# Hanbo-Cheng/DAWN-pytorch

Measured on AMD Instinct MI355X. Metric: generated frames/sec at 256x256, 50 DDIM steps, higher is better.
Workload: dtype f32

## Files before the change

dawn-pytorch_amd/csrc/misc.hip:

```cpp
#include "dawn_common.h"
#include "../../include/dawn_hip.h"

namespace {

__global__ __launch_bounds__(256) void init_conv_x_kernel(const float* __restrict__ x, const float* __restrict__ w3,
                                                          const float* __restrict__ fea_pre, int F, int h, int w,
                                                          int Co, float* __restrict__ out, const long plane) {
    extern __shared__ __attribute__((aligned(16))) float ws[];
    for (int i = threadIdx.x; i < 147 * Co; i += 256) ws[i] = w3[i];
    __syncthreads();
    const int tpp = Co >> 2;
    const long npix = (long)F * h * w;
    const long total = npix * tpp;
    for (long t = (long)blockIdx.x * 256 + threadIdx.x; t < total; t += (long)gridDim.x * 256) {
        const long pix = t / tpp;
        const int cq = (int)(t - pix * tpp);
        const int f = (int)(pix / (h * w));
        const int rem = (int)(pix - (long)f * h * w);
        const int y = rem / w, xx = rem - y * w;
        f32x4 acc = *reinterpret_cast<const f32x4*>(fea_pre + (long)rem * Co + cq * 4);
        for (int ky = 0; ky < 7; ++ky) {
            const int yi = y + ky - 3;
            if (yi < 0 || yi >= h) continue;
            for (int kx = 0; kx < 7; ++kx) {
                const int xi = xx + kx - 3;
                if (xi < 0 || xi >= w) continue;
                const long off = ((long)f * h + yi) * w + xi;
#pragma unroll
                for (int c = 0; c < 3; ++c) {
                    const float xv = x[c * plane + off];
                    const f32x4 wv = *reinterpret_cast<const f32x4*>(ws + ((ky * 7 + kx) * 3 + c) * Co + cq * 4);
                    acc += xv * wv;
                }
            }
        }
        *reinterpret_cast<f32x4*>(out + pix * Co + cq * 4) = acc;
    }
}

__global__ __launch_bounds__(256) void init_conv_x_mfma_kernel(const float* __restrict__ x, const float* __restrict__ w3,
                                                               const float* __restrict__ fea_pre, int F, int h, int w,
                                                               float* __restrict__ out, const long plane) {
    extern __shared__ __attribute__((aligned(16))) float sm[];
    constexpr int Co = 64, KP = 148;
    const int TR = 256 / w, PW = w + 6, PS = (TR + 6) * PW;
    float* Ws = sm;
    float* Ps = sm + KP * Co;
    const int tid = threadIdx.x;
    const int tiles_per_frame = h / TR;
    for (int i = tid; i < KP * Co; i += 256) Ws[i] = i < 147 * Co ? w3[i] : 0.f;
    for (int tile = blockIdx.x; tile < F * tiles_per_frame; tile += gridDim.x) {
    const int f = tile / tiles_per_frame;
    const int y0 = (tile - f * tiles_per_frame) * TR;
    __syncthreads();
    for (int i = tid; i < 3 * PS; i += 256) {
        const int c = i / PS, rem = i - c * PS;
        const int py = rem / PW, px = rem - py * PW;
        const int y = y0 + py - 3, xx = px - 3;
        Ps[i] = (y >= 0 && y < h && xx >= 0 && xx < w) ? x[c * plane + ((long)f * h + y) * w + xx] : 0.f;
    }
    __syncthreads();
    const int wave = tid >> 6, lane = tid & 63, l31 = lane & 31, half = lane >> 5;
    f32x16 acc[2][2];
#pragma unroll
    for (int i = 0; i < 2; ++i)
#pragma unroll
        for (int j = 0; j < 2; ++j)
#pragma unroll
            for (int r = 0; r < 16; ++r) acc[i][j][r] = 0.f;
    int pbase[2];
#pragma unroll
    for (int i = 0; i < 2; ++i) {
        const int p = wave * 64 + i * 32 + l31;
        const int ty = p / w, tx = p - ty * w;
        pbase[i] = ty * PW + tx;
    }
#pragma unroll 2
    for (int s = 0; s < KP / 2; ++s) {
        const int k = 2 * s + half;
        const int kk = k < 147 ? k : 0;
        const int tap = kk / 3, c = kk - tap * 3;
        const int ky = tap / 7, kx = tap - ky * 7;
        const int koff = c * PS + ky * PW + kx;
        const float a0 = Ws[k * Co + l31], a1 = Ws[k * Co + 32 + l31];
        const float b0 = Ps[pbase[0] + koff], b1 = Ps[pbase[1] + koff];
        acc[0][0] = __builtin_amdgcn_mfma_f32_32x32x2f32(a0, b0, acc[0][0], 0, 0, 0);
        acc[0][1] = __builtin_amdgcn_mfma_f32_32x32x2f32(a1, b0, acc[0][1], 0, 0, 0);
        acc[1][0] = __builtin_amdgcn_mfma_f32_32x32x2f32(a0, b1, acc[1][0], 0, 0, 0);
        acc[1][1] = __builtin_amdgcn_mfma_f32_32x32x2f32(a1, b1, acc[1][1], 0, 0, 0);
    }
#pragma unroll
    for (int i = 0; i < 2; ++i) {
        const int p = wave * 64 + i * 32 + l31;
        const long rem = (long)y0 * w + p;
        const float* fp = fea_pre + rem * Co;
        float* op = out + ((long)f * h * w + rem) * Co;
#pragma unroll
        for (int j = 0; j < 2; ++j)
#pragma unroll
            for (int g = 0; g < 4; ++g) {
                const int n = 32 * j + 8 * g + 4 * half;
                const f32x4 v = {acc[i][j][4 * g], acc[i][j][4 * g + 1], acc[i][j][4 * g + 2], acc[i][j][4 * g + 3]};
                *reinterpret_cast<f32x4*>(op + n) = v + *reinterpret_cast<const f32x4*>(fp + n);
            }
    }
    }
}

__global__ __launch_bounds__(256) void head_out_kernel(const float* __restrict__ hg, const float* __restrict__ ho,
                                                       const float* __restrict__ wg, const float* __restrict__ bg,
                                                       const float* __restrict__ wo, const float* __restrict__ bo,
                                                       long rows, int Co, float* __restrict__ eps_out) {
    const int sub = threadIdx.x & 15;
    const long row = (long)blockIdx.x * 16 + (threadIdx.x >> 4);
    float a0 = 0.f, a1 = 0.f, a2 = 0.f;
    if (row < rows) {
        for (int c = sub * 4; c < Co; c += 64) {
            if (hg) {
                const f32x4 g = *reinterpret_cast<const f32x4*>(hg + row * Co + c);
                const f32x4 w0 = *reinterpret_cast<const f32x4*>(wg + c);
                const f32x4 w1 = *reinterpret_cast<const f32x4*>(wg + Co + c);
                a0 += g.x * w0.x + g.y * w0.y + g.z * w0.z + g.w * w0.w;
                a1 += g.x * w1.x + g.y * w1.y + g.z * w1.z + g.w * w1.w;
            }
            if (ho) {
                const f32x4 o = *reinterpret_cast<const f32x4*>(ho + row * Co + c);
                const f32x4 w2 = *reinterpret_cast<const f32x4*>(wo + c);
                a2 += o.x * w2.x + o.y * w2.y + o.z * w2.z + o.w * w2.w;
            }
        }
    }
    a0 = wave_sum(a0, 16); a1 = wave_sum(a1, 16); a2 = wave_sum(a2, 16);
    if (row < rows && sub == 0) {
        if (hg) {
            eps_out[row] = a0 + bg[0];
            eps_out[rows + row] = a1 + bg[1];
        }
        if (ho) eps_out[2 * rows + row] = a2 + bo[0];
    }
}

constexpr int HEADS_RPT = 4;
template <int NQ>
__global__ __launch_bounds__(256) void heads_eps_kernel(const float* __restrict__ c2g, const float* __restrict__ a2g, const float* __restrict__ b2g,
                                                        const float* __restrict__ c2o, const float* __restrict__ a2o, const float* __restrict__ b2o,
                                                        const float* __restrict__ in0, int ld0, int C0, const float* __restrict__ in1, int ld1, int C1,
                                                        const float* __restrict__ wg, const float* __restrict__ wo, const float* __restrict__ Wf,
                                                        const float* __restrict__ bf, long rows, int Co, float* __restrict__ eps_out) {
    const int sub = threadIdx.x & 15;
    const long row0 = (long)blockIdx.x * (16 * HEADS_RPT) + (threadIdx.x >> 4);
    const int Cin = C0 + C1;
    const f32x4 z4 = {0.f, 0.f, 0.f, 0.f};
    f32x4 wg0[NQ], wg1[NQ], wo2[NQ], ag[NQ], bgn[NQ], ao[NQ], bon[NQ], f0[NQ][3], f1[NQ][3];
#pragma unroll
    for (int q = 0; q < NQ; ++q) {
        const int c = sub * 4 + 64 * q;
        wg0[q] = wg1[q] = wo2[q] = ag[q] = bgn[q] = ao[q] = bon[q] = z4;
#pragma unroll
        for (int j = 0; j < 3; ++j) f0[q][j] = f1[q][j] = z4;
// ... 41 lines not shown
                const float sg = dawn_silu(vg[i][q][e] * ag[q][e] + bgn[q][e]);
                const float so = dawn_silu(vo[i][q][e] * ao[q][e] + bon[q][e]);
                const float x0 = v0[i][q][e], x1 = v1[i][q][e];
                e0 += sg * wg0[q][e] + x0 * f0[q][0][e] + x1 * f1[q][0][e];
                e1 += sg * wg1[q][e] + x0 * f0[q][1][e] + x1 * f1[q][1][e];
                e2 += so * wo2[q][e] + x0 * f0[q][2][e] + x1 * f1[q][2][e];
            }
        }
        e0 = wave_sum(e0, 16); e1 = wave_sum(e1, 16); e2 = wave_sum(e2, 16);
        if (row < rows && sub == 0) {
            if (c2g) {
                eps_out[row] = e0 + bf[0];
                eps_out[rows + row] = e1 + bf[1];
            }
            if (c2o) eps_out[2 * rows + row] = e2 + bf[2];
        }
    }
}

__global__ __launch_bounds__(256) void linear_kernel(const float* __restrict__ in, int M, int K, int ld_in,
                                                     const float* __restrict__ W, const float* __restrict__ bias, int N,
                                                     int act_in, float* __restrict__ out, int ld_out) {
    const long o = (long)blockIdx.x * 4 + (threadIdx.x >> 6);
    if (o >= (long)M * N) return;
    const int lane = threadIdx.x & 63;
    const int m = (int)(o / N), n = (int)(o - (long)m * N);
    float acc = 0.f;
    for (int k = lane; k < K; k += 64) {
        float v = in[(long)m * ld_in + k];
        if (act_in == 1) v = dawn_silu(v);
        else if (act_in == 2) v = 0.5f * v * (1.0f + erff(v * 0.70710678118654752f));
        acc += v * W[(long)n * K + k];
    }
    acc = wave_sum(acc);
    if (lane == 0) out[(long)m * ld_out + n] = acc + (bias ? bias[n] : 0.f);
}

__global__ void sinusoidal_kernel(float t, int dim, const float* __restrict__ freqs, float* __restrict__ out) {
    const int i = threadIdx.x;
    const int half = dim / 2;
    if (i < half) {
        const float a = __fmul_rn(t, freqs[i]);
        out[i] = sinf(a);
        out[half + i] = cosf(a);
    }
}

}

extern "C" int dawn_init_conv_x_ex(const float* x, long plane_stride, const float* w3, const float* fea_pre, int F, int h, int w, int Co,
                                   float* out, void* stream) {
    if (plane_stride < (long)F * h * w) return dawn_set_error_msg(-61, "dawn_init_conv_x: plane stride smaller than a plane");
    if (Co % 4 != 0 || 147 * Co * 4 > 60000) return dawn_set_error_msg(-60, "dawn_init_conv_x: bad Co");
    if (Co == 64 && w <= 256 && 256 % w == 0 && h % (256 / w) == 0 && (256 / w) <= h) {
        const int TR = 256 / w;
        const int lds = (148 * 64 + 3 * (TR + 6) * (w + 6)) * (int)sizeof(float);
        const int ntiles = F * (h / TR);
        const int slots = 3 * 256;
        hipLaunchKernelGGL(init_conv_x_mfma_kernel, dim3(ntiles < slots ? ntiles : slots), dim3(256), lds, (hipStream_t)stream, x, w3, fea_pre,
                           F, h, w, out, plane_stride);
        DAWN_LAUNCH_CHECK();
        return 0;
    }
    const long total = (long)F * h * w * (Co / 4);
    int grid = (int)((total + 255) / 256);
    if (grid > 4096) grid = 4096;
    hipLaunchKernelGGL(init_conv_x_kernel, dim3(grid), dim3(256), 147 * Co * sizeof(float), (hipStream_t)stream, x, w3,
                       fea_pre, F, h, w, Co, out, plane_stride);
    DAWN_LAUNCH_CHECK();
    return 0;
}
extern "C" int dawn_init_conv_x(const float* x, const float* w3, const float* fea_pre, int F, int h, int w, int Co,
                                float* out, void* stream) {
    return dawn_init_conv_x_ex(x, (long)F * h * w, w3, fea_pre, F, h, w, Co, out, stream);
}
extern "C" int dawn_head_out(const float* hg, const float* ho, const float* wg, const float* bg, const float* wo,
                             const float* bo, long rows, int Co, float* eps_out, void* stream) {
    hipLaunchKernelGGL(head_out_kernel, dim3(dawn_cdiv(rows, 16)), dim3(256), 0, (hipStream_t)stream, hg, ho, wg, bg,
                       wo, bo, rows, Co, eps_out);
    DAWN_LAUNCH_CHECK();
    return 0;
}
extern "C" int dawn_heads_eps(const float* c2g, const float* a2g, const float* b2g, const float* c2o, const float* a2o, const float* b2o,
                              const float* in0, int ld0, int C0, const float* in1, int ld1, int C1, const float* wg, const float* wo,
                              const float* Wf, const float* bf, long rows, int Co, float* eps_out, void* stream) {
    if (Co <= 0 || Co % 4 != 0 || C0 <= 0 || C0 % 4 != 0 || C1 < 0 || C1 % 4 != 0 || ld0 % 4 != 0 || ld1 % 4 != 0 || ld0 < C0 || ld1 < C1)
        return dawn_set_error_msg(-62, "dawn_heads_eps: Co, C0, C1, ld0 and ld1 must be multiples of 4 (ld >= C)");
    if (Co > 256 || C0 > 256 || C1 > 256) return dawn_set_error_msg(-62, "dawn_heads_eps: more than 256 channels in one source");
    if ((!c2g && !c2o) || !in0 || (C1 > 0 && !in1) || !Wf || !bf || !eps_out || (c2g && (!a2g || !b2g || !wg)) || (c2o && (!a2o || !b2o || !wo)))
        return dawn_set_error_msg(-62, "dawn_heads_eps: null argument");
    const uintptr_t al = (uintptr_t)c2g | (uintptr_t)a2g | (uintptr_t)b2g | (uintptr_t)c2o | (uintptr_t)a2o | (uintptr_t)b2o | (uintptr_t)in0 |
                         (uintptr_t)in1 | (uintptr_t)wg | (uintptr_t)wo | (uintptr_t)Wf;
    if (al & 15) return dawn_set_error_msg(-62, "dawn_heads_eps: pointers must be 16-byte aligned");
    if (rows <= 0) return 0;
    const int mc = Co > C0 ? (Co > C1 ? Co : C1) : (C0 > C1 ? C0 : C1);
    const dim3 grid(dawn_cdiv(rows, 16 * HEADS_RPT)), block(256);
#define HEADS_LAUNCH(NQ)                                                                                                              \
    hipLaunchKernelGGL(heads_eps_kernel<NQ>, grid, block, 0, (hipStream_t)stream, c2g, a2g, b2g, c2o, a2o, b2o, in0, ld0, C0, in1, ld1, C1, \
                       wg, wo, Wf, bf, rows, Co, eps_out)
    if (mc <= 64) HEADS_LAUNCH(1);
    else if (mc <= 128) HEADS_LAUNCH(2);
    else HEADS_LAUNCH(4);
#undef HEADS_LAUNCH
    DAWN_LAUNCH_CHECK();
    return 0;
}
extern "C" int dawn_fold_heads(const float* wg, const float* bg, const float* wo, const float* bo, const float* wr_g, const float* br_g,
                               const float* wr_o, const float* br_o, int Co, int Cin, float* Wf, float* bf) {
    if (!wg || !bg || !wo || !bo || !wr_g || !br_g || !wr_o || !br_o || !Wf || !bf || Co <= 0 || Cin <= 0)
        return dawn_set_error_msg(-63, "dawn_fold_heads: null argument or empty shape");
    for (int j = 0; j < 3; ++j) {
        const float* w = j < 2 ? wg + (long)j * Co : wo;
        const float* wr = j < 2 ? wr_g : wr_o;
// ... 59 lines not shown
```

dawn-pytorch_amd/csrc/sampler.hip:

```cpp
#include "dawn_common.h"
#include "../../include/dawn_hip.h"
#include <stdio.h>

namespace {

__global__ __launch_bounds__(256) void ddim_x0_kernel(const float* __restrict__ x, const float* __restrict__ eps,
                                                      float recip, float recipm1, long n, float* __restrict__ x0,
                                                      unsigned* __restrict__ hist) {
    __shared__ unsigned hs[2048];
    for (int i = threadIdx.x; i < 2048; i += 256) hs[i] = 0;
    __syncthreads();
    for (long i = (long)blockIdx.x * 256 + threadIdx.x; i < n; i += (long)gridDim.x * 256) {
        const float v = __fsub_rn(__fmul_rn(recip, x[i]), __fmul_rn(recipm1, eps[i]));
        x0[i] = v;
        const unsigned u = __float_as_uint(v) & 0x7fffffffu;
        atomicAdd(&hs[u >> 20], 1u);
    }
    __syncthreads();
    for (int i = threadIdx.x; i < 2048; i += 256)
        if (hs[i]) atomicAdd(&hist[i], hs[i]);
}

__global__ __launch_bounds__(256) void select_hist_kernel(const float* __restrict__ x0, long n,
                                                          const unsigned* __restrict__ state, int pass,
                                                          unsigned* __restrict__ hist) {
    __shared__ unsigned hs[1024];
    const unsigned prefix = state[0];
    if (pass < 4) {
        for (int i = threadIdx.x; i < 1024; i += 256) hs[i] = 0;
    } else if (threadIdx.x == 0) {
        hs[0] = 0x7fffffffu;
    }
    __syncthreads();
    const int sh = pass == 2 ? 20 : 10;
    for (long i = (long)blockIdx.x * 256 + threadIdx.x; i < n; i += (long)gridDim.x * 256) {
        const unsigned u = __float_as_uint(x0[i]) & 0x7fffffffu;
        if (pass == 4) {
            if (u > prefix) atomicMin(&hs[0], u);
        } else if ((u >> sh) == prefix) {
            atomicAdd(&hs[(pass == 2 ? (u >> 10) : u) & 1023u], 1u);
        }
    }
    __syncthreads();
    if (pass == 4) {
        if (threadIdx.x == 0) atomicMin(&hist[0], hs[0]);
    } else {
        for (int i = threadIdx.x; i < 1024; i += 256)
            if (hs[i]) atomicAdd(&hist[i], hs[i]);
    }
}

__global__ __launch_bounds__(256) void select_scan_kernel(const unsigned* __restrict__ hist, int nbins,
                                                          unsigned long long rank0, unsigned* __restrict__ state,
                                                          int pass) {
    __shared__ unsigned long long part[256];
    const int per = nbins / 256;
    const int t = threadIdx.x;
    unsigned long long s = 0;
    for (int i = 0; i < per; ++i) s += hist[t * per + i];
    part[t] = s;
    __syncthreads();
    if (t == 0) {
        const unsigned long long r = pass == 1 ? rank0 : (unsigned long long)state[1];
        unsigned long long cum = 0;
        int ch = -1;
        for (int i = 0; i < 256; ++i) {
            if (r < cum + part[i]) { ch = i; break; }
            cum += part[i];
        }
        if (ch < 0) { ch = 255; cum -= part[255]; }
        int b = ch * per + per - 1;
        unsigned long long before = cum;
        for (int i = 0; i < per; ++i) {
            const unsigned long long c = hist[ch * per + i];
            if (r < before + c) { b = ch * per + i; break; }
            if (i < per - 1) before += c;
        }
        const unsigned long long rin = r >= before ? r - before : 0;
        const unsigned prefix = pass == 1 ? 0u : state[0];
        state[0] = pass == 1 ? (unsigned)b : ((prefix << 10) | (unsigned)b);
        state[1] = (unsigned)rin;
        state[2] = hist[b];
        state[3] = (rin + 1 < (unsigned long long)hist[b]) ? 1u : 0u;
    }
}

__global__ void select_finalize_kernel(const unsigned* __restrict__ state, const unsigned* __restrict__ hmin,
                                       float weight, float* __restrict__ s_out) {
    if (threadIdx.x == 0 && blockIdx.x == 0) {
        const float lo = __uint_as_float(state[0]);
        float hi = lo;
        if (!state[3] && hmin[0] != 0x7fffffffu) hi = __uint_as_float(hmin[0]);
        const float df = __fsub_rn(hi, lo);
        float q = weight < 0.5f ? __fadd_rn(lo, __fmul_rn(weight, df)) : __fsub_rn(hi, __fmul_rn(df, __fsub_rn(1.0f, weight)));
        s_out[0] = fmaxf(q, 1.0f);
        s_out[1] = q;
    }
}

__global__ __launch_bounds__(256) void ddim_update_kernel(const float* __restrict__ x0, const float* __restrict__ eps,
                                                          const float* __restrict__ sp, const float* __restrict__ noise,
                                                          float san, float c, float sigma, long n,
                                                          float* __restrict__ x) {
    const float s = sp[0];
    for (long i = (long)blockIdx.x * 256 + threadIdx.x; i < n; i += (long)gridDim.x * 256) {
        float v = fminf(fmaxf(x0[i], -s), s) / s;
        float r = __fadd_rn(__fmul_rn(v, san), __fmul_rn(c, eps[i]));
        if (noise) r = __fadd_rn(r, __fmul_rn(sigma, noise[i]));
        x[i] = r;
    }
}

__global__ __launch_bounds__(256) void ancestral_update_kernel(const float* __restrict__ x0, const float* x_t,
                                                               const float* __restrict__ sp, const float* __restrict__ noise,
                                                               float c1, float c2, float std, long n, float* out) {
    const float s = sp[0];
    for (long i = (long)blockIdx.x * 256 + threadIdx.x; i < n; i += (long)gridDim.x * 256) {
        float v = fminf(fmaxf(x0[i], -s), s) / s;
        float r = __fadd_rn(__fmul_rn(v, c1), __fmul_rn(c2, x_t[i]));
        if (noise) r = __fadd_rn(r, __fmul_rn(std, noise[i]));
        out[i] = r;
    }
}

__device__ __forceinline__ void philox_round(unsigned& c0, unsigned& c1, unsigned& c2, unsigned& c3, unsigned k0,
                                             unsigned k1) {
    const unsigned long long p0 = (unsigned long long)0xD2511F53u * c0;
    const unsigned long long p1 = (unsigned long long)0xCD9E8D57u * c2;
    const unsigned n0 = (unsigned)(p1 >> 32) ^ c1 ^ k0;
    const unsigned n1 = (unsigned)p1;
    const unsigned n2 = (unsigned)(p0 >> 32) ^ c3 ^ k1;
    const unsigned n3 = (unsigned)p0;
    c0 = n0; c1 = n1; c2 = n2; c3 = n3;
}

__global__ __launch_bounds__(256) void philox_normal_kernel(float* __restrict__ out, int C, int F, int f0, int Ftotal,
                                                            int hw, unsigned long long seed, unsigned stream_id) {
    const int qpf = hw >> 2;
    const long total = (long)C * F * qpf;
    for (long t = (long)blockIdx.x * 256 + threadIdx.x; t < total; t += (long)gridDim.x * 256) {
        const int qd = (int)(t % qpf);
        const long cf = t / qpf;
        const int f = (int)(cf % F), c = (int)(cf / F);
        const unsigned long long gq = ((unsigned long long)c * Ftotal + (f0 + f)) * qpf + qd;
        unsigned c0 = (unsigned)gq, c1 = (unsigned)(gq >> 32), c2 = stream_id, c3 = 0x44415757u;
        unsigned k0 = (unsigned)seed, k1 = (unsigned)(seed >> 32);
#pragma unroll
        for (int r = 0; r < 10; ++r) {
            philox_round(c0, c1, c2, c3, k0, k1);
            k0 += 0x9E3779B9u;
            k1 += 0xBB67AE85u;
        }
        const float u0 = ((float)c0 + 0.5f) * 2.3283064365386963e-10f;
        const float u1 = ((float)c1 + 0.5f) * 2.3283064365386963e-10f;
        const float u2 = ((float)c2 + 0.5f) * 2.3283064365386963e-10f;
        const float u3 = ((float)c3 + 0.5f) * 2.3283064365386963e-10f;
        const float r0 = sqrtf(-2.0f * logf(fminf(fmaxf(u0, 1e-10f), 1.0f)));
        const float r1 = sqrtf(-2.0f * logf(fminf(fmaxf(u2, 1e-10f), 1.0f)));
        float s0, c0f, s1, c1f;
        sincosf(6.283185307179586f * u1, &s0, &c0f);
        sincosf(6.283185307179586f * u3, &s1, &c1f);
        f32x4 v = {r0 * c0f, r0 * s0, r1 * c1f, r1 * s1};
        *reinterpret_cast<f32x4*>(out + ((long)c * F + f) * hw + qd * 4) = v;
    }
}

__global__ __launch_bounds__(256) void cfg_combine_kernel(const float* __restrict__ e_null, const float* __restrict__ e_cond,
                                                          float scale, long n, float* __restrict__ out) {
    for (long i = (long)blockIdx.x * 256 + threadIdx.x; i < n; i += (long)gridDim.x * 256)
        out[i] = __fadd_rn(e_null[i], __fmul_rn(__fsub_rn(e_cond[i], e_null[i]), scale));
}

__global__ __launch_bounds__(256) void cfg_x0_kernel(const float* e_null, const float* e_cond, float scale,
                                                     const float* __restrict__ x, float recip, float recipm1, long n,
                                                     float* eps_out, float* __restrict__ x0, unsigned* __restrict__ hist) {
    __shared__ unsigned hs[2048];
    for (int i = threadIdx.x; i < 2048; i += 256) hs[i] = 0;
    __syncthreads();
    for (long i = (long)blockIdx.x * 256 + threadIdx.x; i < n; i += (long)gridDim.x * 256) {
        const float en = e_null[i];
        const float e = __fadd_rn(en, __fmul_rn(__fsub_rn(e_cond[i], en), scale));
        eps_out[i] = e;
        const float v = __fsub_rn(__fmul_rn(recip, x[i]), __fmul_rn(recipm1, e));
        x0[i] = v;
        const unsigned u = __float_as_uint(v) & 0x7fffffffu;
        atomicAdd(&hs[u >> 20], 1u);
    }
    __syncthreads();
    for (int i = threadIdx.x; i < 2048; i += 256)
        if (hs[i]) atomicAdd(&hist[i], hs[i]);
}

__device__ __forceinline__ float step_fixed_one(float xv, float ev, float recip, float recipm1, float a, float b, int clamp,
                                                bool anc, bool has_noise, float sg, float nz, float& x0v) {
#pragma clang fp contract(off)
    x0v = __builtin_fmaf(recip, xv, -(recipm1 * ev));
    const float v = clamp ? fminf(fmaxf(x0v, -1.0f), 1.0f) : x0v;
    float r = (v * a) + (b * (anc ? xv : ev));
    if (has_noise) r = __builtin_fmaf(sg, nz, r);
    return r;
}

template <bool ANC>
__global__ __launch_bounds__(256) void step_fixed_kernel(const float* x, const float* __restrict__ eps,
                                                         const float* __restrict__ noise, float recip, float recipm1, float a,
                                                         float b, float sg, int clamp, long n, int vec,
                                                         float* __restrict__ x0_out, float* out) {
    const long stride = (long)gridDim.x * 256;
    const long n4 = vec ? (n >> 2) : 0;
    for (long i = (long)blockIdx.x * 256 + threadIdx.x; i < n4; i += stride) {
        const f32x4 xv = reinterpret_cast<const f32x4*>(x)[i];
        const f32x4 ev = reinterpret_cast<const f32x4*>(eps)[i];
        f32x4 nv = {0.f, 0.f, 0.f, 0.f};
        if (noise) nv = reinterpret_cast<const f32x4*>(noise)[i];
        f32x4 r, x0v;
#pragma unroll
        for (int k = 0; k < 4; ++k) {
            float t0;
            r[k] = step_fixed_one(xv[k], ev[k], recip, recipm1, a, b, clamp, ANC, noise != nullptr, sg, nv[k], t0);
            x0v[k] = t0;
        }
        if (x0_out) reinterpret_cast<f32x4*>(x0_out)[i] = x0v;
        reinterpret_cast<f32x4*>(out)[i] = r;
    }
    for (long i = n4 * 4 + (long)blockIdx.x * 256 + threadIdx.x; i < n; i += stride) {
        float t0;
        const float t = step_fixed_one(x[i], eps[i], recip, recipm1, a, b, clamp, ANC, noise != nullptr, sg, noise ? noise[i] : 0.f, t0);
        if (x0_out) x0_out[i] = t0;
        out[i] = t;
    }
}

int grid_for(long n) {
    long g = (n + 255) / 256;
    if (g > 2048) g = 2048;
    if (g < 1) g = 1;
    return (int)g;
}

}

extern "C" int dawn_ddim_x0(const float* x, const float* eps, float recip, float recipm1, long n, float* x0,
                            unsigned* hist, void* stream) {
    hipLaunchKernelGGL(ddim_x0_kernel, dim3(grid_for(n)), dim3(256), 0, (hipStream_t)stream, x, eps, recip, recipm1, n,
                       x0, hist);
    DAWN_LAUNCH_CHECK();
    return 0;
}
extern "C" int dawn_select_ws_reset(unsigned* ws, void* stream) {
    hipError_t e = hipMemsetAsync(ws, 0, (size_t)(2048 + 1024 + 1024 + 4) * 4, (hipStream_t)stream);
    if (e == hipSuccess) e = hipMemsetD32Async((hipDeviceptr_t)(ws + 2048 + 1024 + 1024 + 4), 0x7fffffff, 4, (hipStream_t)stream);
    if (e != hipSuccess) return dawn_set_error(e, __FILE__, __LINE__);
    return 0;
}
extern "C" int dawn_select_scan(const unsigned* hist, int nbins, unsigned long long rank, unsigned* state, int pass,
                                void* stream) {
    if (nbins % 256 != 0) return dawn_set_error_msg(-70, "dawn_select_scan: nbins must be a multiple of 256");
    hipLaunchKernelGGL(select_scan_kernel, dim3(1), dim3(256), 0, (hipStream_t)stream, hist, nbins, rank, state, pass);
    DAWN_LAUNCH_CHECK();
    return 0;
}
extern "C" int dawn_select_hist(const float* x0, long n, const unsigned* state, int pass, unsigned* hist,
                                void* stream) {
    if (pass < 2 || pass > 4) return dawn_set_error_msg(-71, "dawn_select_hist: pass must be 2, 3 or 4");
    hipLaunchKernelGGL(select_hist_kernel, dim3(grid_for(n)), dim3(256), 0, (hipStream_t)stream, x0, n, state, pass,
                       hist);
    DAWN_LAUNCH_CHECK();
    return 0;
}
extern "C" int dawn_select_finalize(const unsigned* state, const unsigned* hist3, float weight, float* s_out,
                                    void* stream) {
    hipLaunchKernelGGL(select_finalize_kernel, dim3(1), dim3(64), 0, (hipStream_t)stream, state, hist3, weight, s_out);
    DAWN_LAUNCH_CHECK();
    return 0;
}
extern "C" int dawn_ddim_update(const float* x0, const float* eps, const float* s, const float* noise,
                                float sqrt_alpha_next, float c, float sigma, long n, float* x, void* stream) {
    hipLaunchKernelGGL(ddim_update_kernel, dim3(grid_for(n)), dim3(256), 0, (hipStream_t)stream, x0, eps, s, noise,
                       sqrt_alpha_next, c, sigma, n, x);
    DAWN_LAUNCH_CHECK();
    return 0;
}
extern "C" int dawn_ancestral_update(const float* x0, const float* x_t, const float* s, const float* noise, float c1, float c2,
                                     float std, long n, float* out, void* stream) {
    if (out == x0 || (noise && out == noise))
        return dawn_set_error_msg(-78, "dawn_ancestral_update: out must not alias x0 or noise (out == x_t is allowed)");
    hipLaunchKernelGGL(ancestral_update_kernel, dim3(grid_for(n)), dim3(256), 0, (hipStream_t)stream, x0, x_t, s, noise, c1, c2,
                       std, n, out);
    DAWN_LAUNCH_CHECK();
    return 0;
}
static bool ranges_overlap(const float* p, const float* q, long n) { return p && q && p < q + n && q < p + n; }
static int step_fixed_launch(bool anc, const char* who, const float* x, const float* eps, const float* noise, float recip,
                             float recipm1, float a, float b, float sg, int clamp, long n, float* x0_out, float* out, void* stream) {
    char msg[160];
    if (!x || !eps || !out || n < 0) {
        snprintf(msg, sizeof(msg), "%s: null argument", who);
        return dawn_set_error_msg(-79, msg);
    }
    if (clamp != 0 && clamp != 1) {
        snprintf(msg, sizeof(msg), "%s: clamp must be 1 (static) or 0 (none)", who);
        return dawn_set_error_msg(-79, msg);
    }
    if (anc && !clamp) {
        snprintf(msg, sizeof(msg), "%s: clamp = 0 does not exist for the ancestral step (p_sample always clips, MT:1113)", who);
        return dawn_set_error_msg(-79, msg);
    }
    const bool bad = (out != x && ranges_overlap(out, x, n)) || ranges_overlap(out, eps, n) || ranges_overlap(out, noise, n) ||
                     ranges_overlap(out, x0_out, n) || ranges_overlap(x0_out, x, n) || ranges_overlap(x0_out, eps, n) ||
                     ranges_overlap(x0_out, noise, n);
    if (bad) {
        snprintf(msg, sizeof(msg), "%s: out must not alias eps, noise or x0_out (out == x is allowed); x0_out must not alias an input", who);
        return dawn_set_error_msg(-80, msg);
    }
    if (n == 0) return 0;
    const uintptr_t bits = (uintptr_t)x | (uintptr_t)eps | (uintptr_t)noise | (uintptr_t)x0_out | (uintptr_t)out;
    const int vec = (bits & 15) == 0 && n >= 4;
    const int grid = grid_for(vec ? (n + 3) / 4 : n);
    if (anc)
        hipLaunchKernelGGL(step_fixed_kernel<true>, dim3(grid), dim3(256), 0, (hipStream_t)stream, x, eps, noise, recip, recipm1, a,
                           b, sg, clamp, n, vec, x0_out, out);
    else
        hipLaunchKernelGGL(step_fixed_kernel<false>, dim3(grid), dim3(256), 0, (hipStream_t)stream, x, eps, noise, recip, recipm1, a,
                           b, sg, clamp, n, vec, x0_out, out);
    DAWN_LAUNCH_CHECK();
    return 0;
}
extern "C" int dawn_ddim_step_fixed(const float* x, const float* eps, const float* noise, float recip, float recipm1,
                                    float sqrt_alpha_next, float c, float sigma, int clamp, long n, float* x0_out, float* out,
                                    void* stream) {
    return step_fixed_launch(false, "dawn_ddim_step_fixed", x, eps, noise, recip, recipm1, sqrt_alpha_next, c, sigma, clamp, n, x0_out,
                             out, stream);
}
extern "C" int dawn_ancestral_step_fixed(const float* x_t, const float* eps, const float* noise, float recip, float recipm1, float c1,
                                         float c2, float std, int clamp, long n, float* x0_out, float* out, void* stream) {
    return step_fixed_launch(true, "dawn_ancestral_step_fixed", x_t, eps, noise, recip, recipm1, c1, c2, std, clamp, n, x0_out, out,
                             stream);
}
extern "C" int dawn_cfg_combine(const float* e_null, const float* e_cond, float scale, long n, float* out,
                                void* stream) {
    hipLaunchKernelGGL(cfg_combine_kernel, dim3(grid_for(n)), dim3(256), 0, (hipStream_t)stream, e_null, e_cond, scale,
                       n, out);
    DAWN_LAUNCH_CHECK();
    return 0;
}
extern "C" int dawn_cfg_x0(const float* e_null, const float* e_cond, float scale, const float* x, float recip, float recipm1, long n,
                           float* eps_out, float* x0_out, unsigned* hist1, void* stream) {
    if (x0_out == x || x0_out == eps_out) return dawn_set_error_msg(-73, "dawn_cfg_x0: x0_out must not alias x or eps_out");
    hipLaunchKernelGGL(cfg_x0_kernel, dim3(grid_for(n)), dim3(256), 0, (hipStream_t)stream, e_null, e_cond, scale, x, recip,
                       recipm1, n, eps_out, x0_out, hist1);
    DAWN_LAUNCH_CHECK();
    return 0;
}
extern "C" int dawn_philox_normal(float* out, int C, int F, int f0, int Ftotal, int hw, uint64_t seed,
                                  uint32_t stream_id, void* stream) {
    if (hw % 4 != 0) return dawn_set_error_msg(-72, "dawn_philox_normal: h*w must be a multiple of 4");
    hipLaunchKernelGGL(philox_normal_kernel, dim3(grid_for((long)C * F * (hw / 4))), dim3(256), 0, (hipStream_t)stream,
                       out, C, F, f0, Ftotal, hw, (unsigned long long)seed, stream_id);
    DAWN_LAUNCH_CHECK();
    return 0;
}
```

Baseline: 173.9.

## Use split-bf16 MFMA for init conv and rework x0/histogram selection kernels

Replaces the fp32 MFMA 7x7 input convolution with a version that splits fp32 operands into three bf16 parts and uses 32x32x16 bf16 MFMA. It double-buffers input tiles in LDS and prefetches the next tile while computing the current one. Separately, the sampler's x0/histogram and select kernels move to 1024-thread blocks with vectorized loads, wave-aggregated atomics, per-wave histogram copies and a parallel prefix scan. The intent is to cut the conv's compute cost and reduce atomic contention. In exchange it adds bf16-split numerical error and considerable complexity.

```diff
diff --git a/dawn-pytorch_amd/csrc/misc.hip b/dawn-pytorch_amd/csrc/misc.hip
--- a/dawn-pytorch_amd/csrc/misc.hip
+++ b/dawn-pytorch_amd/csrc/misc.hip
@@ -18,7 +18,7 @@
         const int f = (int)(pix / (h * w));
         const int rem = (int)(pix - (long)f * h * w);
         const int y = rem / w, xx = rem - y * w;
-        f32x4 acc = *reinterpret_cast<const f32x4*>(fea_pre + (long)rem * Co + cq * 4);
+        f32x4 acc = {0.f, 0.f, 0.f, 0.f};
         for (int ky = 0; ky < 7; ++ky) {
             const int yi = y + ky - 3;
             if (yi < 0 || yi >= h) continue;
@@ -34,77 +34,223 @@
                 }
             }
         }
-        *reinterpret_cast<f32x4*>(out + pix * Co + cq * 4) = acc;
-    }
-}
-
-__global__ __launch_bounds__(256) void init_conv_x_mfma_kernel(const float* __restrict__ x, const float* __restrict__ w3,
-                                                               const float* __restrict__ fea_pre, int F, int h, int w,
-                                                               float* __restrict__ out, const long plane) {
-    extern __shared__ __attribute__((aligned(16))) float sm[];
-    constexpr int Co = 64, KP = 148;
-    const int TR = 256 / w, PW = w + 6, PS = (TR + 6) * PW;
-    float* Ws = sm;
-    float* Ps = sm + KP * Co;
+        *reinterpret_cast<f32x4*>(out + pix * Co + cq * 4) = acc + *reinterpret_cast<const f32x4*>(fea_pre + (long)rem * Co + cq * 4);
+    }
+}
+
+constexpr int IC_KS = 11;
+constexpr int IC_WPLANE = IC_KS * 2 * 64 * 16;
+constexpr int IC_MAXQ = 6;
+typedef unsigned ic_u32x4 __attribute__((ext_vector_type(4)));
+typedef unsigned ic_u32x2 __attribute__((ext_vector_type(2)));
+
+__device__ __forceinline__ f32x16 mfma32(const dawn_bf16x8 a, const dawn_bf16x8 b, const f32x16 c) {
+    f32x16 d = __builtin_amdgcn_mfma_f32_32x32x16_bf16(a, b, c, 0, 0, 0);
+    asm("" : "+a"(d) : "v"(a), "v"(b));
+    return d;
+}
+__device__ __forceinline__ void ic_split3_quad(const f32x4 v, uint2& p1, uint2& p2, uint2& p3) {
+    unsigned q1[2], q2[2], q3[2];
+#pragma unroll
+    for (int i = 0; i < 2; ++i) {
+        const float a = v[2 * i], b = v[2 * i + 1];
+        const unsigned a1 = __float_as_uint(a) & 0xffff0000u, b1 = __float_as_uint(b) & 0xffff0000u;
+        const float ra = a - __uint_as_float(a1), rb = b - __uint_as_float(b1);
+        const unsigned a2 = __float_as_uint(ra) & 0xffff0000u, b2 = __float_as_uint(rb) & 0xffff0000u;
+        const float sa = ra - __uint_as_float(a2), sb = rb - __uint_as_float(b2);
+        q1[i] = __builtin_amdgcn_perm(b1, a1, 0x07060302u);
+        q2[i] = __builtin_amdgcn_perm(b2, a2, 0x07060302u);
+        q3[i] = __builtin_amdgcn_perm(__float_as_uint(sb), __float_as_uint(sa), 0x07060302u);
+    }
+    p1 = uint2{q1[0], q1[1]};
+    p2 = uint2{q2[0], q2[1]};
+    p3 = uint2{q3[0], q3[1]};
+}
+template <int JJ>
+__device__ __forceinline__ dawn_bf16x8 ic_frag(const unsigned (&d)[6]) {
+    ic_u32x4 r;
+    if constexpr (JJ == 0) {
+#pragma unroll
+        for (int k = 0; k < 4; ++k) r[k] = __builtin_amdgcn_alignbit(d[k + 1], d[k], 16);
+    } else if constexpr (JJ == 1) {
+        r = ic_u32x4{d[1], d[2], d[3], d[4]};
+    } else if constexpr (JJ == 2) {
+#pragma unroll
+        for (int k = 0; k < 4; ++k) r[k] = __builtin_amdgcn_alignbit(d[k + 2], d[k + 1], 16);
+    } else {
+        r = ic_u32x4{d[2], d[3], d[4], d[5]};
+    }
+    return __builtin_bit_cast(dawn_bf16x8, r);
+}
+
+__global__ __launch_bounds__(256) void init_conv_x_split_kernel(const float* __restrict__ x, const float* __restrict__ w3,
+                                                                const float* __restrict__ fea_pre, int F, int h, int w,
+                                                                float* __restrict__ out, const long plane, const int vec) {
+    extern __shared__ __attribute__((aligned(16))) unsigned char smb[];
+    constexpr int Co = 64;
+    const int TR = 256 / w, PR = TR + 6, PWp = w + 8, NCH = w / 4 + 2;
+    const int PLB = 3 * PR * PWp * 2;
+    unsigned char* Wl = smb;
+    unsigned char* Pl = smb + 3 * IC_WPLANE;
     const int tid = threadIdx.x;
     const int tiles_per_frame = h / TR;
-    for (int i = tid; i < KP * Co; i += 256) Ws[i] = i < 147 * Co ? w3[i] : 0.f;
-    for (int tile = blockIdx.x; tile < F * tiles_per_frame; tile += gridDim.x) {
-    const int f = tile / tiles_per_frame;
-    const int y0 = (tile - f * tiles_per_frame) * TR;
+    const int ntiles = F * tiles_per_frame;
+
+    for (int i = tid; i < 2 * IC_KS * Co; i += 256) {
+        const int rr = i >> 6, co = i & 63;
+        const int c = rr / 7, ky = rr - 7 * c;
+        float v[8];
+#pragma unroll
+        for (int kx = 0; kx < 8; ++kx) v[kx] = (rr < 21 && kx < 7) ? w3[((ky * 7 + kx) * 3 + c) * Co + co] : 0.f;
+        dawn_bf16x8 p1, p2, p3;
+        dawn_split3_oct(v, p1, p2, p3);
+        unsigned char* dst = Wl + (rr * Co + co) * 16;
+        *reinterpret_cast<dawn_bf16x8*>(dst) = p1;
+        *reinterpret_cast<dawn_bf16x8*>(dst + IC_WPLANE) = p2;
+        *reinterpret_cast<dawn_bf16x8*>(dst + 2 * IC_WPLANE) = p3;
+    }
+
+    int q_dst[IC_MAXQ], q_row[IC_MAXQ], q_rel[IC_MAXQ], q_c[IC_MAXQ];
+#pragma unroll
+    for (int i = 0; i < IC_MAXQ; ++i) {
+        const int u = tid + 256 * i;
+        const int c = u / (PR * NCH), r2 = u - c * (PR * NCH);
+        const int prow = r2 / NCH, q = r2 - prow * NCH;
+        const bool pad = q == 0 || q == NCH - 1;
+        q_dst[i] = u < 3 * PR * NCH ? ((c * PR + prow) * PWp + 4 * q) * 2 : -1;
+        q_row[i] = pad ? -(1 << 20) : prow;
+        q_rel[i] = prow * w + 4 * (q - 1);
+        q_c[i] = c < 3 ? c : 0;
+    }
+    f32x4 raw[IC_MAXQ];
+    unsigned okm = 0;
+    auto fetch = [&](int tile) {
+        const int f = tile / tiles_per_frame;
+        const int y0 = (tile - f * tiles_per_frame) * TR;
+        const long tb = ((long)f * h + y0 - 3) * w;
+        okm = 0;
+#pragma unroll
+        for (int i = 0; i < IC_MAXQ; ++i) {
+            const int y = y0 - 3 + q_row[i];
+            const bool ok = q_dst[i] >= 0 && y >= 0 && y < h;
+            okm |= ok ? (1u << i) : 0u;
+            const float* p = ok ? x + (q_c[i] * plane + tb + q_rel[i]) : x;
+            if (vec) raw[i] = *reinterpret_cast<const f32x4*>(p);
+            else raw[i] = f32x4{p[0], p[1], p[2], p[3]};
+        }
+    };
+    auto spill = [&](unsigned char* Pb) {
+#pragma unroll
+        for (int i = 0; i < IC_MAXQ; ++i) {
+            if (q_dst[i] >= 0) {
+                const f32x4 v = (okm >> i & 1u) ? raw[i] : f32x4{0.f, 0.f, 0.f, 0.f};
+                uint2 p1, p2, p3;
+                ic_split3_quad(v, p1, p2, p3);
+                *reinterpret_cast<uint2*>(Pb + q_dst[i]) = p1;
+                *reinterpret_cast<uint2*>(Pb + PLB + q_dst[i]) = p2;
+                *reinterpret_cast<uint2*>(Pb + 2 * PLB + q_dst[i]) = p3;
+            }
+        }
+    };
+
+    const int lane = tid & 63, l31 = lane & 31, half = lane >> 5;
+    const int wave = __builtin_amdgcn_readfirstlane(tid >> 6);
+    const int cw = wave & 1, jw = wave >> 1;
+    const int G = w >> 3;
+    const int m = l31 & (G - 1), ty = l31 / G;
+    const int bB = (ty * PWp + 8 * m + 4 * jw) * 2;
+    const int aA = (half * Co + cw * 32 + l31) * 16;
+    int roff[IC_KS];
+#pragma unroll
+    for (int s = 0; s < IC_KS; ++s) {
+        const int rr = 2 * s + half;
+        const int c = rr / 7, ky = rr - 7 * c;
+        roff[s] = rr < 21 ? (c * PR + ky) * PWp * 2 : 0;
+    }
+#define REGION() __builtin_amdgcn_sched_barrier(0)
+
+    if ((int)blockIdx.x < ntiles) {
+        fetch(blockIdx.x);
+        spill(Pl);
+    }
     __syncthreads();
-    for (int i = tid; i < 3 * PS; i += 256) {
-        const int c = i / PS, rem = i - c * PS;
-        const int py = rem / PW, px = rem - py * PW;
-        const int y = y0 + py - 3, xx = px - 3;
-        Ps[i] = (y >= 0 && y < h && xx >= 0 && xx < w) ? x[c * plane + ((long)f * h + y) * w + xx] : 0.f;
-    }
-    __syncthreads();
-    const int wave = tid >> 6, lane = tid & 63, l31 = lane & 31, half = lane >> 5;
-    f32x16 acc[2][2];
-#pragma unroll
-    for (int i = 0; i < 2; ++i)
-#pragma unroll
-        for (int j = 0; j < 2; ++j)
-#pragma unroll
-            for (int r = 0; r < 16; ++r) acc[i][j][r] = 0.f;
-    int pbase[2];
-#pragma unroll
-    for (int i = 0; i < 2; ++i) {
-        const int p = wave * 64 + i * 32 + l31;
-        const int ty = p / w, tx = p - ty * w;
-        pbase[i] = ty * PW + tx;
-    }
-#pragma unroll 2
-    for (int s = 0; s < KP / 2; ++s) {
-        const int k = 2 * s + half;
-        const int kk = k < 147 ? k : 0;
-        const int tap = kk / 3, c = kk - tap * 3;
-        const int ky = tap / 7, kx = tap - ky * 7;
-        const int koff = c * PS + ky * PW + kx;
-        const float a0 = Ws[k * Co + l31], a1 = Ws[k * Co + 32 + l31];
-        const float b0 = Ps[pbase[0] + koff], b1 = Ps[pbase[1] + koff];
-        acc[0][0] = __builtin_amdgcn_mfma_f32_32x32x2f32(a0, b0, acc[0][0], 0, 0, 0);
-        acc[0][1] = __builtin_amdgcn_mfma_f32_32x32x2f32(a1, b0, acc[0][1], 0, 0, 0);
-        acc[1][0] = __builtin_amdgcn_mfma_f32_32x32x2f32(a0, b1, acc[1][0], 0, 0, 0);
-        acc[1][1] = __builtin_amdgcn_mfma_f32_32x32x2f32(a1, b1, acc[1][1], 0, 0, 0);
-    }
-#pragma unroll
-    for (int i = 0; i < 2; ++i) {
-        const int p = wave * 64 + i * 32 + l31;
-        const long rem = (long)y0 * w + p;
-        const float* fp = fea_pre + rem * Co;
-        float* op = out + ((long)f * h * w + rem) * Co;
-#pragma unroll
-        for (int j = 0; j < 2; ++j)
+    int it = 0;
+    for (int tile = blockIdx.x; tile < ntiles; tile += gridDim.x, ++it) {
+        const int f = tile / tiles_per_frame;
+        const int y0 = (tile - f * tiles_per_frame) * TR;
+        const unsigned char* Pb = Pl + (it & 1) * 3 * PLB;
+        const bool more = tile + (int)gridDim.x < ntiles;
+        if (more) fetch(tile + gridDim.x);
+        f32x4 fpv[4][4];
+        long orow[4];
+#pragma unroll
+        for (int jj = 0; jj < 4; ++jj) {
+            const long rem = (long)(y0 + ty) * w + 8 * m + 4 * jw + jj;
+            orow[jj] = ((long)f * h * w + rem) * Co + cw * 32 + 4 * half;
+#pragma unroll
+            for (int g = 0; g < 4; ++g) fpv[jj][g] = *reinterpret_cast<const f32x4*>(fea_pre + rem * Co + cw * 32 + 4 * half + 8 * g);
+        }
+        f32x16 acc[4];
+#pragma unroll
+        for (int jj = 0; jj < 4; ++jj)
+#pragma unroll
+            for (int r = 0; r < 16; ++r) acc[jj][r] = 0.f;
+        dawn_bf16x8 fa[2][3];
+        unsigned fd[2][3][6];
+        auto frags = [&](int s, int buf) {
+#pragma unroll
+            for (int pl = 0; pl < 3; ++pl) {
+                fa[buf][pl] = *reinterpret_cast<const dawn_bf16x8*>(Wl + pl * IC_WPLANE + s * (2 * Co * 16) + aA);
+                const unsigned char* bp = Pb + pl * PLB + roff[s] + bB;
+#pragma unroll
+                for (int t = 0; t < 3; ++t) {
+                    const ic_u32x2 d2 = *reinterpret_cast<const ic_u32x2*>(__builtin_assume_aligned(bp + 8 * t, 8));
+                    fd[buf][pl][2 * t] = d2[0];
+                    fd[buf][pl][2 * t + 1] = d2[1];
+                }
+            }
+        };
+        REGION();
+        frags(0, 0);
+        REGION();
+#pragma unroll
+        for (int s = 0; s < IC_KS; ++s) {
+            const int cur = s & 1;
+            if (s + 1 < IC_KS) frags(s + 1, cur ^ 1);
+            REGION();
+            dawn_bf16x8 fb[4][3];
+#pragma unroll
+            for (int pl = 0; pl < 3; ++pl) {
+                asm volatile("" : "+v"(fa[cur][pl]), "+v"(fd[cur][pl][0]), "+v"(fd[cur][pl][1]), "+v"(fd[cur][pl][2]), "+v"(fd[cur][pl][3]),
+                                  "+v"(fd[cur][pl][4]), "+v"(fd[cur][pl][5]));
+                fb[0][pl] = ic_frag<0>(fd[cur][pl]);
+                fb[1][pl] = ic_frag<1>(fd[cur][pl]);
+                fb[2][pl] = ic_frag<2>(fd[cur][pl]);
+                fb[3][pl] = ic_frag<3>(fd[cur][pl]);
+            }
+            constexpr int PW6[6] = {0, 2, 1, 0, 1, 0};
+            constexpr int PX6[6] = {2, 0, 1, 1, 0, 0};
+#pragma unroll
+            for (int u = 0; u < 6; ++u)
+#pragma unroll
+                for (int jj = 0; jj < 4; ++jj) acc[jj] = mfma32(fa[cur][PW6[u]], fb[jj][PX6[u]], acc[jj]);
+            const float cl = (acc[0][0] + acc[1][0]) + (acc[2][0] + acc[3][0]);
+            asm volatile("" :: "v"(cl));
+            REGION();
+        }
+        if (more) spill(Pl + ((it & 1) ^ 1) * 3 * PLB);
+#pragma unroll
+        for (int jj = 0; jj < 4; ++jj)
 #pragma unroll
             for (int g = 0; g < 4; ++g) {
-                const int n = 32 * j + 8 * g + 4 * half;
-                const f32x4 v = {acc[i][j][4 * g], acc[i][j][4 * g + 1], acc[i][j][4 * g + 2], acc[i][j][4 * g + 3]};
-                *reinterpret_cast<f32x4*>(op + n) = v + *reinterpret_cast<const f32x4*>(fp + n);
-            }
-    }
-    }
+                const f32x4 v = {acc[jj][4 * g], acc[jj][4 * g + 1], acc[jj][4 * g + 2], acc[jj][4 * g + 3]};
+                *reinterpret_cast<f32x4*>(out + orow[jj] + 8 * g) = v + fpv[jj][g];
+            }
+        asm volatile("s_waitcnt lgkmcnt(0)" ::: "memory");
+        __builtin_amdgcn_s_barrier();
+        asm volatile("" ::: "memory");
+    }
+#undef REGION
 }
 
 __global__ __launch_bounds__(256) void head_out_kernel(const float* __restrict__ hg, const float* __restrict__ ho,
@@ -252,13 +398,15 @@
                                    float* out, void* stream) {
     if (plane_stride < (long)F * h * w) return dawn_set_error_msg(-61, "dawn_init_conv_x: plane stride smaller than a plane");
     if (Co % 4 != 0 || 147 * Co * 4 > 60000) return dawn_set_error_msg(-60, "dawn_init_conv_x: bad Co");
-    if (Co == 64 && w <= 256 && 256 % w == 0 && h % (256 / w) == 0 && (256 / w) <= h) {
+    if (Co == 64 && w >= 8 && w <= 256 && 256 % w == 0 && h % (256 / w) == 0 && (256 / w) <= h) {
         const int TR = 256 / w;
-        const int lds = (148 * 64 + 3 * (TR + 6) * (w + 6)) * (int)sizeof(float);
+        const int lds = 3 * IC_WPLANE + 2 * 3 * (3 * (TR + 6) * (w + 8) * 2);
         const int ntiles = F * (h / TR);
-        const int slots = 3 * 256;
-        hipLaunchKernelGGL(init_conv_x_mfma_kernel, dim3(ntiles < slots ? ntiles : slots), dim3(256), lds, (hipStream_t)stream, x, w3, fea_pre,
-                           F, h, w, out, plane_stride);
+        const int slots = 256;
+        const int vec = (((uintptr_t)x & 15) == 0 && (plane_stride & 3) == 0) ? 1 : 0;
+        (void)hipFuncSetAttribute((const void*)init_conv_x_split_kernel, hipFuncAttributeMaxDynamicSharedMemorySize, lds);
+        hipLaunchKernelGGL(init_conv_x_split_kernel, dim3(ntiles < slots ? ntiles : slots), dim3(256), lds, (hipStream_t)stream, x, w3, fea_pre,
+                           F, h, w, out, plane_stride, vec);
         DAWN_LAUNCH_CHECK();
         return 0;
     }
diff --git a/dawn-pytorch_amd/csrc/sampler.hip b/dawn-pytorch_amd/csrc/sampler.hip
--- a/dawn-pytorch_amd/csrc/sampler.hip
+++ b/dawn-pytorch_amd/csrc/sampler.hip
@@ -4,80 +4,175 @@
 
 namespace {
 
-__global__ __launch_bounds__(256) void ddim_x0_kernel(const float* __restrict__ x, const float* __restrict__ eps,
-                                                      float recip, float recipm1, long n, float* __restrict__ x0,
+constexpr int SEL_THREADS = 1024;
+constexpr int HIST_AGG_ROUNDS = 4;
+__device__ __forceinline__ void wave_hist_add(unsigned* __restrict__ hw, unsigned bin, bool on) {
+    unsigned long long todo = __ballot(on);
+    const int lane = threadIdx.x & 63;
+#pragma unroll
+    for (int r = 0; r < HIST_AGG_ROUNDS; ++r) {
+        if (!todo) break;
+        const int leader = __ffsll((long long)todo) - 1;
+        const unsigned b = (unsigned)__builtin_amdgcn_readlane((int)bin, leader);
+        const bool hit = on && bin == b;
+        const unsigned long long same = __ballot(hit);
+        if (lane == leader) atomicAdd(&hw[b], (unsigned)__popcll(same));
+        todo &= ~same;
+        on = on && !hit;
+    }
+    if (on) atomicAdd(&hw[bin], 1u);
+}
+
+__device__ __forceinline__ float x0_one(float xv, float ev, float recip, float recipm1) {
+#pragma clang fp contract(off)
+    return __builtin_fmaf(recip, xv, -(recipm1 * ev));
+}
+__device__ __forceinline__ float cfg_one(float en, float ec, float scale) {
+#pragma clang fp contract(off)
+    return __builtin_fmaf(ec - en, scale, en);
+}
+
+template <bool CFG>
+__device__ __forceinline__ void x0_hist_body(const float* e_null, const float* eps_in, float scale, const float* __restrict__ x, float recip,
+                                             float recipm1, long n, int vec, float* eps_out, float* __restrict__ x0,
+                                             unsigned* __restrict__ hist, unsigned* hs) {
+    for (int i = threadIdx.x; i < 4 * 2048; i += SEL_THREADS) hs[i] = 0;
+    __syncthreads();
+    unsigned* hw = hs + ((threadIdx.x >> 6) & 3) * 2048;
+    const long stride = (long)gridDim.x * SEL_THREADS;
+    const long n4 = vec ? (n >> 2) : 0;
+    for (long base = (long)blockIdx.x * SEL_THREADS; base < n4; base += stride) {
+        const long i = base + threadIdx.x;
+        const bool on = i < n4;
+        f32x4 v = {0.f, 0.f, 0.f, 0.f};
+        if (on) {
+            const f32x4 xv = reinterpret_cast<const f32x4*>(x)[i];
+            f32x4 ev = reinterpret_cast<const f32x4*>(eps_in)[i];
+            if (CFG) {
+                const f32x4 nv = reinterpret_cast<const f32x4*>(e_null)[i];
+#pragma unroll
+                for (int k = 0; k < 4; ++k) ev[k] = cfg_one(nv[k], ev[k], scale);
+                reinterpret_cast<f32x4*>(eps_out)[i] = ev;
+            }
+#pragma unroll
+            for (int k = 0; k < 4; ++k) v[k] = x0_one(xv[k], ev[k], recip, recipm1);
+            reinterpret_cast<f32x4*>(x0)[i] = v;
+        }
+#pragma unroll
+        for (int k = 0; k < 4; ++k) wave_hist_add(hw, (__float_as_uint(v[k]) & 0x7fffffffu) >> 20, on);
+    }
+    for (long base = n4 * 4 + (long)blockIdx.x * SEL_THREADS; base < n; base += stride) {
+        const long i = base + threadIdx.x;
+        const bool on = i < n;
+        float v = 0.f;
+        if (on) {
+            float ev = eps_in[i];
+            if (CFG) {
+                ev = cfg_one(e_null[i], ev, scale);
+                eps_out[i] = ev;
+            }
+            v = x0_one(x[i], ev, recip, recipm1);
+            x0[i] = v;
+        }
+        wave_hist_add(hw, (__float_as_uint(v) & 0x7fffffffu) >> 20, on);
+    }
+    __syncthreads();
+    for (int i = threadIdx.x; i < 2048; i += SEL_THREADS) {
+        const unsigned c = (hs[i] + hs[2048 + i]) + (hs[4096 + i] + hs[6144 + i]);
+        if (c) atomicAdd(&hist[i], c);
+    }
+}
+
+__global__ __launch_bounds__(SEL_THREADS) void ddim_x0_kernel(const float* __restrict__ x, const float* __restrict__ eps,
+                                                      float recip, float recipm1, long n, int vec, float* __restrict__ x0,
                                                       unsigned* __restrict__ hist) {
-    __shared__ unsigned hs[2048];
-    for (int i = threadIdx.x; i < 2048; i += 256) hs[i] = 0;
-    __syncthreads();
-    for (long i = (long)blockIdx.x * 256 + threadIdx.x; i < n; i += (long)gridDim.x * 256) {
-        const float v = __fsub_rn(__fmul_rn(recip, x[i]), __fmul_rn(recipm1, eps[i]));
-        x0[i] = v;
-        const unsigned u = __float_as_uint(v) & 0x7fffffffu;
-        atomicAdd(&hs[u >> 20], 1u);
-    }
-    __syncthreads();
-    for (int i = threadIdx.x; i < 2048; i += 256)
-        if (hs[i]) atomicAdd(&hist[i], hs[i]);
-}
-
-__global__ __launch_bounds__(256) void select_hist_kernel(const float* __restrict__ x0, long n,
+    __shared__ unsigned hs[4 * 2048];
+    x0_hist_body<false>(nullptr, eps, 0.f, x, recip, recipm1, n, vec, nullptr, x0, hist, hs);
+}
+
+__global__ __launch_bounds__(SEL_THREADS) void select_hist_kernel(const float* __restrict__ x0, long n, int vec,
                                                           const unsigned* __restrict__ state, int pass,
                                                           unsigned* __restrict__ hist) {
-    __shared__ unsigned hs[1024];
+    __shared__ unsigned hs[4 * 1024];
     const unsigned prefix = state[0];
     if (pass < 4) {
-        for (int i = threadIdx.x; i < 1024; i += 256) hs[i] = 0;
+        for (int i = threadIdx.x; i < 4 * 1024; i += SEL_THREADS) hs[i] = 0;
     } else if (threadIdx.x == 0) {
         hs[0] = 0x7fffffffu;
     }
     __syncthreads();
+    unsigned* hw = hs + ((threadIdx.x >> 6) & 3) * 1024;
     const int sh = pass == 2 ? 20 : 10;
-    for (long i = (long)blockIdx.x * 256 + threadIdx.x; i < n; i += (long)gridDim.x * 256) {
-        const unsigned u = __float_as_uint(x0[i]) & 0x7fffffffu;
+    unsigned mn = 0x7fffffffu;
+    auto one = [&](unsigned u, bool on) {
         if (pass == 4) {
-            if (u > prefix) atomicMin(&hs[0], u);
-        } else if ((u >> sh) == prefix) {
-            atomicAdd(&hs[(pass == 2 ? (u >> 10) : u) & 1023u], 1u);
-        }
-    }
-    __syncthreads();
+            if (on && u > prefix && u < mn) mn = u;
+        } else {
+            wave_hist_add(hw, (pass == 2 ? (u >> 10) : u) & 1023u, on && (u >> sh) == prefix);
+        }
+    };
+    const long stride = (long)gridDim.x * SEL_THREADS;
+    const long n4 = vec ? (n >> 2) : 0;
+    for (long base = (long)blockIdx.x * SEL_THREADS; base < n4; base += stride) {
+        const long i = base + threadIdx.x;
+        const bool on = i < n4;
+        f32x4 v = {0.f, 0.f, 0.f, 0.f};
+        if (on) v = reinterpret_cast<const f32x4*>(x0)[i];
+#pragma unroll
+        for (int k = 0; k < 4; ++k) one(__float_as_uint(v[k]) & 0x7fffffffu, on);
+    }
+    for (long base = n4 * 4 + (long)blockIdx.x * SEL_THREADS; base < n; base += stride) {
+        const long i = base + threadIdx.x;
+        const bool on = i < n;
+        one(on ? __float_as_uint(x0[i]) & 0x7fffffffu : 0u, on);
+    }
     if (pass == 4) {
+#pragma unroll
+        for (int o = 32; o >= 1; o >>= 1) {
+            const unsigned t = (unsigned)__shfl_xor((int)mn, o, 64);
+            mn = t < mn ? t : mn;
+        }
+        if ((threadIdx.x & 63) == 0) atomicMin(&hs[0], mn);
+        __syncthreads();
         if (threadIdx.x == 0) atomicMin(&hist[0], hs[0]);
     } else {
-        for (int i = threadIdx.x; i < 1024; i += 256)
-            if (hs[i]) atomicAdd(&hist[i], hs[i]);
+        __syncthreads();
+        for (int i = threadIdx.x; i < 1024; i += SEL_THREADS) {
+            const unsigned c = (hs[i] + hs[1024 + i]) + (hs[2048 + i] + hs[3072 + i]);
+            if (c) atomicAdd(&hist[i], c);
+        }
     }
 }
 
 __global__ __launch_bounds__(256) void select_scan_kernel(const unsigned* __restrict__ hist, int nbins,
                                                           unsigned long long rank0, unsigned* __restrict__ state,
                                                           int pass) {
-    __shared__ unsigned long long part[256];
+    __shared__ unsigned long long wtot[4];
     const int per = nbins / 256;
-    const int t = threadIdx.x;
+    const int t = threadIdx.x, lane = t & 63, wave = t >> 6;
+    const unsigned long long r = pass == 1 ? rank0 : (unsigned long long)state[1];
+    const unsigned prefix = pass == 1 ? 0u : state[0];
     unsigned long long s = 0;
     for (int i = 0; i < per; ++i) s += hist[t * per + i];
-    part[t] = s;
+    unsigned long long incl = s;
+#pragma unroll
+    for (int o = 1; o < 64; o <<= 1) {
+        const unsigned long long up = __shfl_up(incl, o, 64);
+        if (lane >= o) incl += up;
+    }
+    if (lane == 63) wtot[wave] = incl;
     __syncthreads();
-    if (t == 0) {
-        const unsigned long long r = pass == 1 ? rank0 : (unsigned long long)state[1];
-        unsigned long long cum = 0;
-        int ch = -1;
-        for (int i = 0; i < 256; ++i) {
-            if (r < cum + part[i]) { ch = i; break; }
-            cum += part[i];
-        }
-        if (ch < 0) { ch = 255; cum -= part[255]; }
-        int b = ch * per + per - 1;
+    for (int j = 0; j < wave; ++j) incl += wtot[j];
+    const unsigned long long cum = incl - s;
+    if (t == 255 ? r >= cum : (r >= cum && r < incl)) {
+        int b = t * per + per - 1;
         unsigned long long before = cum;
         for (int i = 0; i < per; ++i) {
-            const unsigned long long c = hist[ch * per + i];
-            if (r < before + c) { b = ch * per + i; break; }
+            const unsigned long long c = hist[t * per + i];
+            if (r < before + c) { b = t * per + i; break; }
             if (i < per - 1) before += c;
         }
         const unsigned long long rin = r >= before ? r - before : 0;
-        const unsigned prefix = pass == 1 ? 0u : state[0];
         state[0] = pass == 1 ? (unsigned)b : ((prefix << 10) | (unsigned)b);
         state[1] = (unsigned)rin;
         state[2] = hist[b];
@@ -171,24 +266,11 @@
         out[i] = __fadd_rn(e_null[i], __fmul_rn(__fsub_rn(e_cond[i], e_null[i]), scale));
 }
 
-__global__ __launch_bounds__(256) void cfg_x0_kernel(const float* e_null, const float* e_cond, float scale,
-                                                     const float* __restrict__ x, float recip, float recipm1, long n,
+__global__ __launch_bounds__(SEL_THREADS) void cfg_x0_kernel(const float* e_null, const float* e_cond, float scale,
+                                                     const float* __restrict__ x, float recip, float recipm1, long n, int vec,
                                                      float* eps_out, float* __restrict__ x0, unsigned* __restrict__ hist) {
-    __shared__ unsigned hs[2048];
-    for (int i = threadIdx.x; i < 2048; i += 256) hs[i] = 0;
-    __syncthreads();
-    for (long i = (long)blockIdx.x * 256 + threadIdx.x; i < n; i += (long)gridDim.x * 256) {
-        const float en = e_null[i];
-        const float e = __fadd_rn(en, __fmul_rn(__fsub_rn(e_cond[i], en), scale));
-        eps_out[i] = e;
-        const float v = __fsub_rn(__fmul_rn(recip, x[i]), __fmul_rn(recipm1, e));
-        x0[i] = v;
-        const unsigned u = __float_as_uint(v) & 0x7fffffffu;
-        atomicAdd(&hs[u >> 20], 1u);
-    }
-    __syncthreads();
-    for (int i = threadIdx.x; i < 2048; i += 256)
-        if (hs[i]) atomicAdd(&hist[i], hs[i]);
+    __shared__ unsigned hs[4 * 2048];
+    x0_hist_body<true>(e_null, e_cond, scale, x, recip, recipm1, n, vec, eps_out, x0, hist, hs);
 }
 
 __device__ __forceinline__ float step_fixed_one(float xv, float ev, float recip, float recipm1, float a, float b, int clamp,
@@ -237,13 +319,23 @@
     if (g < 1) g = 1;
     return (int)g;
 }
+int grid_sel(long n, int vec) {
+    const long chunks = ((vec ? (n + 3) / 4 : n) + SEL_THREADS - 1) / SEL_THREADS;
+    if (chunks <= 1) return 1;
+    const long trips = (chunks + 255) / 256;
+    return (int)((chunks + trips - 1) / trips);
+}
+int all_aligned16(const void* a, const void* b, const void* c, const void* d, const void* e, const void* f) {
+    return (((uintptr_t)a | (uintptr_t)b | (uintptr_t)c | (uintptr_t)d | (uintptr_t)e | (uintptr_t)f) & 15) == 0;
+}
 
 }
 
 extern "C" int dawn_ddim_x0(const float* x, const float* eps, float recip, float recipm1, long n, float* x0,
                             unsigned* hist, void* stream) {
-    hipLaunchKernelGGL(ddim_x0_kernel, dim3(grid_for(n)), dim3(256), 0, (hipStream_t)stream, x, eps, recip, recipm1, n,
-                       x0, hist);
+    const int vec = n >= 4 && all_aligned16(x, eps, x0, nullptr, nullptr, nullptr);
+    hipLaunchKernelGGL(ddim_x0_kernel, dim3(grid_sel(n, vec)), dim3(SEL_THREADS), 0, (hipStream_t)stream, x, eps, recip, recipm1, n,
+                       vec, x0, hist);
     DAWN_LAUNCH_CHECK();
     return 0;
 }
@@ -263,7 +355,8 @@
 extern "C" int dawn_select_hist(const float* x0, long n, const unsigned* state, int pass, unsigned* hist,
                                 void* stream) {
     if (pass < 2 || pass > 4) return dawn_set_error_msg(-71, "dawn_select_hist: pass must be 2, 3 or 4");
-    hipLaunchKernelGGL(select_hist_kernel, dim3(grid_for(n)), dim3(256), 0, (hipStream_t)stream, x0, n, state, pass,
+    const int vec = n >= 4 && all_aligned16(x0, nullptr, nullptr, nullptr, nullptr, nullptr);
+    hipLaunchKernelGGL(select_hist_kernel, dim3(grid_sel(n, vec)), dim3(SEL_THREADS), 0, (hipStream_t)stream, x0, n, vec, state, pass,
                        hist);
     DAWN_LAUNCH_CHECK();
     return 0;
@@ -347,8 +440,9 @@
 extern "C" int dawn_cfg_x0(const float* e_null, const float* e_cond, float scale, const float* x, float recip, float recipm1, long n,
                            float* eps_out, float* x0_out, unsigned* hist1, void* stream) {
     if (x0_out == x || x0_out == eps_out) return dawn_set_error_msg(-73, "dawn_cfg_x0: x0_out must not alias x or eps_out");
-    hipLaunchKernelGGL(cfg_x0_kernel, dim3(grid_for(n)), dim3(256), 0, (hipStream_t)stream, e_null, e_cond, scale, x, recip,
-                       recipm1, n, eps_out, x0_out, hist1);
+    const int vec = n >= 4 && all_aligned16(e_null, e_cond, x, eps_out, x0_out, nullptr);
+    hipLaunchKernelGGL(cfg_x0_kernel, dim3(grid_sel(n, vec)), dim3(SEL_THREADS), 0, (hipStream_t)stream, e_null, e_cond, scale, x, recip,
+                       recipm1, n, vec, eps_out, x0_out, hist1);
     DAWN_LAUNCH_CHECK();
     return 0;
 }
```

Result: no change. 175.3, median of 6 (+0.8%).
